# Christine8888/PsrSigSim

Hardware: AMD Instinct MI355X
Metric: channel-samples/sec (node) at 2048ch x 2^22 samp; % HBM roofline; speedup vs CPU (higher is better)
Workload: dtype f32

## Files before the change

psrsigsim_amd/csrc/pss_fourstep.hip:

```cpp
#include "pss_fourstep.hpp"

using namespace pss;

SideStreams *side_streams() {
    static SideStreams g[64];
    int dev = 0;
    if (hipGetDevice(&dev) != hipSuccess || dev < 0 || dev >= 64) return nullptr;
    SideStreams &x = g[dev];
    if (!x.ok) {
        for (int i = 0; i < 2; ++i)
            if (hipStreamCreateWithFlags(&x.s[i], hipStreamNonBlocking) != hipSuccess) return nullptr;
        for (int i = 0; i < 40; ++i)
            if (hipEventCreateWithFlags(&x.ev[i], hipEventDisableTiming) != hipSuccess) return nullptr;
        x.ok = true;
    }
    return &x;
}

__global__ __launch_bounds__(256) void k_mask_bits(KP k, uint32_t *bm) {
    const int r = blockIdx.y;
    const uint32_t j = blockIdx.x * 256u + threadIdx.x;
    const uint32_t wm = ((uint32_t)k.N - 1u) >> 5;
    if (j > wm) return;
    uint32_t is;
    float t;
    mask_split((uint64_t)k.p.mask_ramp[r], k.log2n, is, t);
    const uint32_t B = (uint32_t)k.mbB, RUN = B < 32u ? B : 32u;
    const uint32_t N1 = (uint32_t)k.N1, N2 = (uint32_t)k.N2;
    uint32_t out = 0;
    for (uint32_t s = 0; s < 32u; s += RUN) {
        const uint32_t bp = (j << 5) + s, e = bp / B, b = bp - e * B;
        const uint32_t n = (e % N1) * N2 + (e / N1) * B + b;
        out |= mask_run(k, n, is, t, RUN) << s;
    }
    bm[(int64_t)r * (wm + 1u) + j] = out;
}

__global__ __launch_bounds__(256) void k_mask_words(const uint2 *bits, uint32_t nwords, uint32_t *list,
                                                    uint32_t *count) {
    const uint32_t w = blockIdx.x * 256u + threadIdx.x;
    bool nz = false;
    if (w < nwords) {
        const uint2 b = bits[w];
        nz = (b.x | b.y) != 0u;
    }
    const uint64_t bal = __ballot(nz);
    const int lane = threadIdx.x & 63;
    uint32_t b0 = 0;
    if (lane == 0 && bal) b0 = atomicAdd(count, (uint32_t)__popcll(bal));
    b0 = __shfl(b0, 0);
    if (nz) list[b0 + (uint32_t)__popcll(bal & ((1ull << lane) - 1ull))] = w;
}

__global__ __launch_bounds__(256) void k_null_fix_list(KP k) {
    __shared__ uint32_t desc[4][64 * 9];
    __shared__ uint32_t dbase[4][64 * 9];
    const int r = blockIdx.y, lane = threadIdx.x & 63, wv = threadIdx.x >> 6;
    const PssPipeline &p = k.p;
    const uint32_t nl = *k.nwlist;
    const uint32_t nm = (uint32_t)k.N - 1u;
    uint32_t is;
    float t;
    mask_split((uint64_t)p.mask_ramp[r], k.log2n, is, t);
    const uint32_t c = (uint32_t)(p.chan0 + r);
    float *row = p.data + (int64_t)r * p.ld;
    const Rng gn(p.seed, p.call_noise, P_NOISE), gr(p.seed, p.call_null, P_REP);
    const float nn = p.noise_norm, sc = p.null_rep_scale;
    const uint32_t stride = gridDim.x * 256u;
    for (uint32_t i0 = blockIdx.x * 256u; i0 < nl; i0 += stride) {
        const uint32_t i = i0 + threadIdx.x;
        uint32_t hits = 0, n0 = 0;
        if (i < nl) {
            const uint32_t w = k.wlist[i];
            n0 = ((w << 5) + is) & nm;
            hits = mask_run(k, n0, is, t, 32u);
        }
        if (__ballot(hits != 0u) == 0ull) continue;
        const uint32_t a = n0 & 3u;
        const uint64_t hx = (uint64_t)hits << a;
        uint32_t cnt = 0;
#pragma unroll
        for (int g = 0; g < 9; ++g) cnt += ((uint32_t)(hx >> (4 * g)) & 15u) ? 1u : 0u;
        const uint64_t below = (1ull << lane) - 1ull;
        uint32_t e = 0, total = 0;
#pragma unroll
        for (int bit = 0; bit < 4; ++bit) {
            const uint64_t bal = __ballot((cnt >> bit) & 1u);
            e += (uint32_t)__popcll(bal & below) << bit;
            total += (uint32_t)__popcll(bal) << bit;
        }
#pragma unroll
        for (int g = 0; g < 9; ++g) {
            const uint32_t h = (uint32_t)(hx >> (4 * g)) & 15u;
            if (h) {
                desc[wv][e] = h;
                dbase[wv][e] = ((n0 - a) + 4u * (uint32_t)g) & nm;
                ++e;
            }
        }
        __builtin_amdgcn_fence(__ATOMIC_RELEASE, "wavefront");
        __builtin_amdgcn_wave_barrier();
        __builtin_amdgcn_fence(__ATOMIC_ACQUIRE, "wavefront");
        for (uint32_t e = (uint32_t)lane; e < total; e += 64u) {
            const uint32_t h = desc[wv][e], nb = dbase[wv][e];
            PSS_DASSERT((int64_t)nb + 4 <= k.N && (nb & 3u) == 0u);
            const float4 xn = chi2_1x4(gn.bits(nb >> 2, c, 0u));
            const float4 xr = chi2_1x4(gr.bits(nb >> 2, c, 0u));
            const float vn[4] = {xn.x, xn.y, xn.z, xn.w}, vr[4] = {xr.x, xr.y, xr.z, xr.w};
            if (h == 15u) {
                *reinterpret_cast<float4 *>(row + nb) =
                    make_float4(fmaf(nn, vn[0], vr[0] * sc), fmaf(nn, vn[1], vr[1] * sc),
                                fmaf(nn, vn[2], vr[2] * sc), fmaf(nn, vn[3], vr[3] * sc));
                continue;
            }
#pragma unroll
            for (int q = 0; q < 4; ++q)
                if ((h >> q) & 1u) row[nb + q] = fmaf(nn, vn[q], vr[q] * sc);
        }
        __builtin_amdgcn_fence(__ATOMIC_RELEASE, "wavefront");
        __builtin_amdgcn_wave_barrier();
        __builtin_amdgcn_fence(__ATOMIC_ACQUIRE, "wavefront");
    }
}

__global__ void k_node_params(uint64_t *ramp, float *nyq, int L) {
    const int j = threadIdx.x;
    if (j < KCH) {
        const double t = cospi((j + 0.5) / KCH);
        const double f = 0.5 * (t + 1.0);
        ramp[j] = (uint64_t)ldexp(f, 64 - L);
        nyq[j] = (float)cospi(f);
    }
}

__global__ __launch_bounds__(256) void k_mask_table(const float *nodes, int64_t N, uint2 *bits,
                                                    uint32_t *base, float *coef, uint32_t *counter) {
    __shared__ float T[KCH * KCH];
    if (threadIdx.x < KCH * KCH) {
        const int n = threadIdx.x / KCH, j = threadIdx.x - n * KCH;
        T[threadIdx.x] = (float)(cospi((double)n * (j + 0.5) / KCH) * (n ? 2.0 : 1.0) / KCH);
    }
    __syncthreads();
    const int64_t p = (int64_t)blockIdx.x * blockDim.x + threadIdx.x;
    float v[KCH], c[KCH];
#pragma unroll
    for (int j = 0; j < KCH; ++j) v[j] = nodes[(int64_t)j * N + p];
    float S = 0.f;
#pragma unroll
    for (int n = 0; n < KCH; ++n) {
        float s = 0.f;
#pragma unroll
        for (int j = 0; j < KCH; ++j) s = fmaf(T[n * KCH + j], v[j], s);
        c[n] = s;
        if (n) S += fabsf(s);
    }
    const float eps = 1e-3f + 4e-6f * (fabsf(c[0]) + S);
    const bool hi = c[0] - S > 1.0f + eps;
    const bool amb = !hi && !(c[0] + S < 1.0f - eps);
// ... 22 lines not shown
    for (uint32_t idx = blockIdx.x * 256u + threadIdx.x; idx < na; idx += gridDim.x * 256u) {
        float4 *dst = reinterpret_cast<float4 *>(coef + (int64_t)idx * KREC);
        const float4 q[3] = {dst[1], dst[2], dst[3]};
        const float c[KCH] = {q[0].x, q[0].y, q[0].z, q[0].w, q[1].x, q[1].y, q[1].z, q[1].w,
                              q[2].x, q[2].y, q[2].z, q[2].w};
        float S = 0.f;
#pragma unroll
        for (int n = 1; n < KCH; ++n) S += fabsf(c[n]);
        float D2 = 0.f;
#pragma unroll
        for (int n = 2; n < KCH; ++n) {
            const float n2 = (float)(n * n);
            D2 = fmaf(n2 * (n2 - 1.0f) * (1.0f / 3.0f), fabsf(c[n]), D2);
        }
        const float err = 4e-6f * (fabsf(c[0]) + S);
        constexpr int NG = 256;
        constexpr float H = 2.0f / NG;
        float rt[10];
#pragma unroll
        for (int i = 0; i < 10; ++i) rt[i] = INFINITY;
        float gprev = cheb_eval_r(q, -1.0f) - 1.0f;
        bool prev = gprev > 0.0f;
        const bool s0 = prev;
        bool cert = true;
        int cnt = 0;
        int jf[10];
#pragma unroll
        for (int i = 0; i < 10; ++i) jf[i] = 0;
        for (int jg = 1; jg <= NG; ++jg) {
            const float tg = -1.0f + (float)jg * H;
            const float g = cheb_eval_r(q, tg) - 1.0f;
            const bool cur = g > 0.0f;
            if (cur != prev) {
                cert = cert && (fabsf(g - gprev) - 2.0f * err > D2 * H * H);
#pragma unroll
                for (int i = 0; i < 10; ++i) if (i == cnt) jf[i] = jg;
                ++cnt;
            } else {
                cert = cert && (fminf(fabsf(g), fabsf(gprev)) - err > D2 * H * H * 0.125f);
            }
            prev = cur;
            gprev = g;
        }
        const int nb = cnt < 10 ? cnt : 10;
#pragma unroll
        for (int i = 0; i < 10; ++i) {
            if (i < nb) {
                const bool pv = (i & 1) ? !s0 : s0;
                float lo = -1.0f + (float)(jf[i] - 1) * H, hi = -1.0f + (float)jf[i] * H;
                for (int it = 0; it < 24; ++it) {
                    const float mid = 0.5f * (lo + hi);
                    if ((cheb_eval_r(q, mid) > 1.0f) == pv) lo = mid; else hi = mid;
                }
                rt[i] = lo;
            }
        }
        if (cert && cnt <= 10) {
            dst[0] = make_float4((float)cnt, s0 ? 1.0f : 0.0f, rt[0], rt[1]);
            dst[1] = make_float4(rt[2], rt[3], rt[4], rt[5]);
            dst[2] = make_float4(rt[6], rt[7], rt[8], rt[9]);
        } else {
            dst[0] = make_float4(-1.0f, 0.0f, 0.0f, 0.0f);
            dst[1] = q[0];
            dst[2] = q[1];
            dst[3] = q[2];
        }
    }
}

int launch_node_params(uint64_t *ramp, float *nyq, int L, hipStream_t st) {
    k_node_params<<<1, 64, 0, st>>>(ramp, nyq, L);
    LAUNCHCHK();
    return PSS_OK;
}
int launch_mask_table(const float *nodes, int64_t N, uint2 *bits, uint32_t *base, float *coef, uint32_t *counter,
                      hipStream_t st) {
    k_mask_table<<<dim3((unsigned)(N / 256)), dim3(256), 0, st>>>(nodes, N, bits, base, coef, counter);
    LAUNCHCHK();
    const unsigned gr = (unsigned)std::min<int64_t>(N / 256, 1024);
    k_mask_roots<<<dim3(gr), dim3(256), 0, st>>>(coef, counter);
    LAUNCHCHK();
    return PSS_OK;
}
int launch_mask_words(const uint2 *bits, uint32_t nwords, uint32_t *list, uint32_t *count, hipStream_t st) {
    k_mask_words<<<dim3((nwords + 255) / 256), dim3(256), 0, st>>>(bits, nwords, list, count);
    LAUNCHCHK();
    return PSS_OK;
}
int launch_mask_bits(const KP &k, uint32_t *bm, hipStream_t st) {
    k_mask_bits<<<dim3((unsigned)((k.N / 32 + 255) / 256), (unsigned)k.p.nchan), dim3(256), 0, st>>>(k, bm);
    LAUNCHCHK();
    return PSS_OK;
}
int launch_null_fix(const KP &k, hipStream_t st) {
    tk_begin(TK_NULLFIX, st);
    const unsigned gx = (unsigned)((k.N / 32 / 8 + 255) / 256);
    k_null_fix_list<<<dim3(gx ? gx : 1, (unsigned)k.p.nchan), dim3(256), 0, st>>>(k);
    tk_end(st);
    LAUNCHCHK();
    return PSS_OK;
}

int run_fourstep(KP &k, hipStream_t st, const float *mask_row) {
    if (!fourstep_split(k.N, plan_variant(k.p) == 0, &k.N1, &k.N2))
        return fail(PSS_EUNSUPPORTED, "four-step: N=%lld", (long long)k.N);
    plan_note("fourstep");
    if (k.N1 == 1024 && k.N2 == 4096) {
        return launch_pair<Pow2Split<1024, 4096>>(k, st, mask_row);
    }
    return run_fourstep_b(k, st, mask_row);
}
```

psrsigsim_amd/csrc/pss_fourstep.hpp:

```cpp
#pragma once
#include "pss_stages.hpp"
#include "pss_fft.hpp"


template <int N1, int B, int T, typename FWD>
struct Cols;

template <int N1, int B, int T, int... F>
struct Cols<N1, B, T, RList<F...>> {
    using FF = Fft<N1, B, T>;
    static constexpr int E = FF::E;
    static constexpr int RF0 = FF::template first<F...>();
    static constexpr int RFL = FF::template last_of<F...>();

    __device__ static void passA(const KP &k) {
        __shared__ cf lds[B * Lds<N1>::RS];
        const int tid = threadIdx.x;
        const int r = blockIdx.y;
        const int64_t n20 = (int64_t)blockIdx.x * B;
        const int64_t N2 = k.N2;
        const bool re_in = k.p.data_in_fft != 0;
        for (int it = tid; it < N1 * B / 4; it += T) {
            const int n1 = it / (B / 4);
            const int b4 = (it - n1 * (B / 4)) * 4;
// ... 830 lines not shown
        const uint32_t RP = (uint32_t)rpitch(k);
        const uint32_t s0 = (uint32_t)n20 * 8u;
        {
#pragma unroll 1
        for (int it = tid; it < N1 * B / 4; it += T) {
            const int k1 = it / (B / 4);
            const int b4 = (it - k1 * (B / 4)) * 4;
            const uint32_t off = ((uint32_t)k1 * RP + (uint32_t)b4) * 8u;
            const float4 lo = Y.ld4(off, s0), hi = Y.ld4(off + 16u, s0);
            const cf a[4] = {make_float2(lo.x, lo.y), make_float2(lo.z, lo.w),
                             make_float2(hi.x, hi.y), make_float2(hi.z, hi.w)};
            const uint32_t m0 = (uint32_t)(n20 + b4) * (uint32_t)k1;
            float r0 = (float)m0 * invN;
            if (r0 >= 0.5f) r0 -= 1.0f;
            float r1 = (float)k1 * invN;
            if (r1 >= 0.5f) r1 -= 1.0f;
            const cf w0 = expi_rev(r0), w1 = expi_rev(r1);
            const cf w2 = cmul(w1, w1);
            const cf tw[4] = {w0, cmul(w0, w1), cmul(w0, w2), cmul(w0, cmul(w2, w1))};
#pragma unroll
            for (int i = 0; i < 4; ++i) {
                lds[LdsC::at(b4 + i, k1)] = cmul(a[i], tw[i]);
            }
        }
        }
        __syncthreads();
        cf v[E];
        if constexpr (kWaveCols) {
            const int wv = tid >> 6, lane = tid & 63;
            cf *wl = lds + wv * LdsC::RS;
            FW::template load<RI0>(v, wl, lane);
            stage_sync<true>();
            FW::template run_tw<true, 1, I...>(v, wl, lane, tw16);
            FW::template store<RIL>(v, wl, lane);
        } else {
            FF::template load<RI0>(v, lds, tid);
            __syncthreads();
            FF::template run_tw<true, 1, I...>(v, lds, tid, tw16);
            FF::template store<RIL>(v, lds, tid);
        }
        __syncthreads();
    }

    __device__ static void passC(const KP &k) {
        __shared__ __align__(128) cf lds[B * LdsC::RS];
        const int tid = threadIdx.x;
        int cbx, pr;
        xcd_block(cbx, pr);
        const int ra = 2 * pr - k.poff, rb = ra + 1;
        const bool hasa = ra >= 0, hasb = rb < k.p.nchan;
        const int64_t n20 = (int64_t)cbx * B;
        const bool mask = k.mtab != 0;
        const float invN = k.invN;
        if constexpr (kRegCols) {
            cf x[N1];
            reg_unspill(k, x, pr, n20 + tid);
#pragma unroll
            for (int n1 = 0; n1 < N1; ++n1) lds[LdsC::at(tid, n1)] = x[n1];
            __syncthreads();
        } else {
            inv_block(k, k.Yd + (int64_t)pr * pstride(k), n20, lds, tid);
        }
#pragma unroll 1
        for (int it = tid; it < N1 * B / 4; it += T) {
            const int n1 = it / (B / 4);
            const int b4 = (it - n1 * (B / 4)) * 4;
            const int64_t n = n1 * k.N2 + n20 + b4;
            float da[4], db[4], ma[4], mb[4];
            const uint32_t ha = (mask && hasa) ? mask_bits4<B, N1>(k, ra, cbx, n1, b4) : 0u;
            const uint32_t hb = (mask && hasb) ? mask_bits4<B, N1>(k, rb, cbx, n1, b4) : 0u;
#pragma unroll
            for (int i = 0; i < 4; ++i) {
                const cf z = lds[LdsC::at(b4 + i, n1)];
                da[i] = z.x * invN;
                db[i] = z.y * invN;
                ma[i] = ((ha >> i) & 1u) ? 2.0f : 0.0f;
                mb[i] = ((hb >> i) & 1u) ? 2.0f : 0.0f;
            }
            if (hasa) epilogue4(k, ra, n, 4, da, ma, false);
            if (hasb) epilogue4(k, rb, n, 4, db, mb, false);
        }
    }

    __device__ static void passC_fast32(const KP &k) {
        static_assert((N1 == 1024 || N1 == 2048) && (T == 1024 || T == 512) && B % (T / 64) == 0 &&
                      kWaveCols == false, "register-resident wide pass C: 2^m columns of 1024 / 2048");
        constexpr int NW = T / 64, CPW = B / NW;
        constexpr int E1 = N1 / 64;
        constexpr int H = N1 / 2;
        constexpr int RSH = H + H / 16 + 1;
        constexpr int OSP = B + 1;
        using LW = Lds<N1, -1>;
        using FWC = Fft<N1, 1, 64, true, -1>;
        constexpr int RI0 = FWC::template first<I...>();
        constexpr int LRI = N1 / RI0;
        constexpr int B1 = B * RSH * 8, B2 = NW * LW::RS * 8, B3 = N1 * OSP * 4;
        constexpr int BUF = (B1 > B2 ? B1 : B2) > B3 ? (B1 > B2 ? B1 : B2) : B3;
        __shared__ __align__(16) char smem[BUF];
        __shared__ cf tw16[kTw16Size];
        const int tid = threadIdx.x, wv = tid >> 6, lane = tid & 63;
        tw16_fill(tw16, tid, T);
        int cbx, pr;
        xcd_block(cbx, pr);
        const int ra = 2 * pr - k.poff, rb = ra + 1;
        const bool hasa = ra >= 0, hasb = rb < k.p.nchan;
        const int64_t N2 = k.N2;
        const PssPipeline &p = k.p;
        const float invN = k.invN, nn = p.noise_norm;
        const int64_t n20 = (int64_t)cbx * B;
        const Buf Y(k.Yd + (int64_t)pr * pstride(k), (uint32_t)(pstride(k) * 8));
        const uint32_t RP = (uint32_t)rpitch(k);
        cf *hb = reinterpret_cast<cf *>(smem);
        cf v[CPW][E1];
        auto fresh = [](int x) __attribute__((always_inline)) { return N1 == 1024 ? opaque(x) : x; };
#pragma unroll
        for (int h = 0; h < 2; ++h) {
            if (h) __syncthreads();
#pragma unroll 1
            for (int it = tid; it < H * B / 4; it += T) {
                const int k1l = it / (B / 4), b4 = (it - k1l * (B / 4)) * 4;
                const int k1 = h * H + k1l;
                const uint32_t off = ((uint32_t)k1 * RP + (uint32_t)b4) * 8u, so = (uint32_t)n20 * 8u;
                const float4 lo = Y.ld4(off, so), hi = Y.ld4(off + 16u, so);
                const cf a[4] = {make_float2(lo.x, lo.y), make_float2(lo.z, lo.w),
                                 make_float2(hi.x, hi.y), make_float2(hi.z, hi.w)};
                const uint32_t m0 = (uint32_t)(n20 + b4) * (uint32_t)k1;
                float r0 = (float)m0 * invN;
                if (r0 >= 0.5f) r0 -= 1.0f;
                float r1 = (float)k1 * invN;
                if (r1 >= 0.5f) r1 -= 1.0f;
                const cf w0 = expi_rev(r0), w1 = expi_rev(r1);
                const cf w2 = cmul(w1, w1);
                const cf tw[4] = {w0, cmul(w0, w1), cmul(w0, w2), cmul(w0, cmul(w2, w1))};
#pragma unroll
                for (int i = 0; i < 4; ++i) hb[(b4 + i) * RSH + k1l + (k1l >> 4)] = cmul(a[i], tw[i]);
            }
            __syncthreads();
#pragma unroll
            for (int i = 0; i < E1; ++i) {
                const int pc = 64 * (i / RI0) + LRI * (i % RI0);
                if (pc / H != h) continue;
                const int pl = lane + pc - h * H;
#pragma unroll
                for (int c = 0; c < CPW; ++c) v[c][i] = hb[(wv + NW * c) * RSH + pl + (pl >> 4)];
            }
        }
        __syncthreads();
        {
            cf *wl = reinterpret_cast<cf *>(smem) + wv * LW::RS;
#pragma unroll
            for (int c = 0; c < CPW; ++c) {
                if (c) stage_sync<true>();
                FWC::template run_tw<true, 1, I...>(v[c], wl, fresh(lane), tw16);
            }
        }
        constexpr int RIL = FWC::template last_of<I...>();
        float *stg = reinterpret_cast<float *>(smem);
        const uint32_t ca = (uint32_t)(p.chan0 + ra), cb = ca + 1u;
        const Rng gn(p.seed, p.call_noise, P_NOISE);
        const uint32_t rbytes = (uint32_t)(k.N * 4);
#pragma unroll
        for (int ch = 0; ch < 2; ++ch) {
            __syncthreads();
            const int sl = fresh(lane);
#pragma unroll
            for (int i = 0; i < E1; ++i) {
                int bb, pos;
                FWC::template where<RIL>(i, sl, bb, pos);
#pragma unroll
                for (int c = 0; c < CPW; ++c) stg[pos * OSP + wv + NW * c] = (ch ? v[c][i].y : v[c][i].x) * invN;
            }
            __syncthreads();
            const bool has = ch ? hasb : hasa;
            if (!has) continue;
            const uint32_t c = ch ? cb : ca;
            const Buf o(p.data + (int64_t)(ch ? rb : ra) * p.ld, rbytes);
            const int t0 = fresh(tid);
#pragma unroll
            for (int t = 0; t < N1 * B / 4 / T; ++t) {
                const int it = t0 + t * T;
                const int n1 = it / (B / 4), c4 = (it - n1 * (B / 4)) * 4;
                const uint32_t n = (uint32_t)(n1 * (int)N2) + (uint32_t)n20 + (uint32_t)c4;
                const float4 x = chi2_1x4(gn.bits(n >> 2, c, 0u));
                const float *sr = stg + n1 * OSP + c4;
                o.st4(fmaf(nn, x.x, sr[0]), fmaf(nn, x.y, sr[1]), fmaf(nn, x.z, sr[2]), fmaf(nn, x.w, sr[3]),
                      n * 4u, 0);
            }
        }
    }

    __device__ static void passC_fast(const KP &k) {
        static_assert(kItemsExact, "fast pass C: whole items per thread");
        __shared__ __align__(128) cf lds[B * LdsC::RS];
        const int tid = threadIdx.x;
        int cbx, pr;
        xcd_block(cbx, pr);
        const int ra = 2 * pr - k.poff, rb = ra + 1;
        const bool hasa = ra >= 0, hasb = rb < k.p.nchan;
        const int64_t N2 = k.N2;
        const PssPipeline &p = k.p;
        const float invN = k.invN, nn = p.noise_norm;
        const uint32_t ca = (uint32_t)(p.chan0 + ra), cb = ca + 1u;
        const Rng gn(p.seed, p.call_noise, P_NOISE);
        const uint32_t rbytes = (uint32_t)(k.N * 4);
        const Buf oa(p.data + (int64_t)max(ra, 0) * p.ld, rbytes), ob(p.data + (int64_t)min(rb, p.nchan - 1) * p.ld, rbytes);
        const int64_t n20 = (int64_t)cbx * B;
        if constexpr (kRegCols) {
            cf x[N1];
            reg_unspill(k, x, pr, n20 + tid);
#pragma unroll
            for (int n1 = 0; n1 < N1; ++n1) lds[LdsC::at(tid, n1)] = x[n1];
            __syncthreads();
        } else {
            inv_block(k, k.Yd + (int64_t)pr * pstride(k), n20, lds, tid);
        }
        float acc[ITEMS][2][4];
#pragma unroll
        for (int t = 0; t < ITEMS; ++t) {
            const int it = tid + t * T;
            const int n1 = it / (B / 4);
            const int b4 = (it - n1 * (B / 4)) * 4;
            const uint32_t n = (uint32_t)(n1 * (int)N2) + (uint32_t)n20 + (uint32_t)b4;
            const float4 xa = chi2_1x4(gn.bits(n >> 2, ca, 0u));
            const float4 xb = chi2_1x4(gn.bits(n >> 2, cb, 0u));
            const float na[4] = {xa.x, xa.y, xa.z, xa.w}, nb[4] = {xb.x, xb.y, xb.z, xb.w};
#pragma unroll
            for (int i = 0; i < 4; ++i) {
                const cf z = lds[LdsC::at(b4 + i, n1)];
                acc[t][0][i] = fmaf(nn, na[i], z.x * invN);
                acc[t][1][i] = fmaf(nn, nb[i], z.y * invN);
            }
        }
#pragma unroll
        for (int t = 0; t < ITEMS; ++t) {
            const int it = tid + t * T;
            const int n1 = it / (B / 4);
            const int b4 = (it - n1 * (B / 4)) * 4;
            const uint32_t off = ((uint32_t)(n1 * (int)N2) + (uint32_t)n20 + (uint32_t)b4) * 4u;
            if (hasa) oa.st4(acc[t][0][0], acc[t][0][1], acc[t][0][2], acc[t][0][3], off, 0);
            if (hasb) ob.st4(acc[t][1][0], acc[t][1][1], acc[t][1][2], acc[t][1][3], off, 0);
        }
    }

    __device__ static void node_col(const KP &k, float *nodes) {
        __shared__ __align__(128) cf lds[B * LdsC::RS];
        const int tid = threadIdx.x;
        int cbx, pr;
        xcd_block(cbx, pr);
        const int64_t n20 = (int64_t)cbx * B;
        const float invN = k.invN;
        inv_block(k, k.Ym + (int64_t)pr * pstride(k), n20, lds, tid);
        float *ra = nodes + (int64_t)(2 * pr) * k.N, *rb = ra + k.N;
        for (int it = tid; it < N1 * B / 4; it += T) {
            const int n1 = it / (B / 4);
            const int b4 = (it - n1 * (B / 4)) * 4;
            const int64_t n = n1 * k.N2 + n20 + b4;
            float a[4], b[4];
#pragma unroll
            for (int i = 0; i < 4; ++i) {
                const cf z = lds[LdsC::at(b4 + i, n1)];
                a[i] = z.x * invN;
                b[i] = z.y * invN;
            }
            *reinterpret_cast<float4 *>(ra + n) = make_float4(a[0], a[1], a[2], a[3]);
            *reinterpret_cast<float4 *>(rb + n) = make_float4(b[0], b[1], b[2], b[3]);
        }
    }
};

template <typename C, int T>
__global__ __launch_bounds__(T) void k_pairA(KP k) { C::template passA<false>(k); }
template <typename C, int T, bool SHARED>
__global__ __launch_bounds__(T) void k_pairA_fast(KP k) { C::template passA<true, SHARED>(k); }
template <typename C>
__global__ __launch_bounds__(256) void k_prof_cols(KP k, float4 *out) { C::prof_cols(k, out); }
template <typename C, int T>
__global__ __launch_bounds__(T) void k_pairC(KP k) { C::passC(k); }
template <typename C, int T>
__global__ __launch_bounds__(T) void k_pairC_fast(KP k) { C::passC_fast(k); }
template <typename C, int T, int W = (T == 512 ? 2 : 4)>
__global__ __launch_bounds__(T, W) void k_pairC_fast32(KP k) { C::passC_fast32(k); }
template <typename C, int T>
__global__ __launch_bounds__(T) void k_node_col(KP k, float *nodes) { C::node_col(k, nodes); }
template <typename C, int T>
__global__ __launch_bounds__(T, C::kFoldWaves) void k_pairA_fold(KP k) { C::passA_fold(k); }
template <typename C, int T>
__global__ __launch_bounds__(T, C::kFoldWavesC) void k_pairC_fold(KP k) { C::passC_fold(k); }

constexpr int xrs_read(int B) { return B >= 32 ? 1 : 16; }

template <int N1_, int B_, int T_, typename CF, typename CI>
struct ColEngine {
    static constexpr int N1 = N1_, B = B_, T = T_;
    using PC = PairCols<N1, B, T, CF, CI, xrs_read(B)>;
    using PCFast = PairCols<N1, B, T, CF, CI, -1>;
    using PCFast32 = PairCols<N1, 16, 512, CF, CI, -1>;
    static constexpr int FB = B > 128 ? 128 : B;
    using PCFold = PairCols<N1, FB, FB, CF, CI>;
    using PCNode = PairCols<N1, B, T, CF, CI>;
    using MaskCols = Cols<N1, B, T, CF>;
};
template <int N1>
struct Pow2Cols;
template <> struct Pow2Cols<16> : ColEngine<16, 512, 512, C16, C16> {};
template <> struct Pow2Cols<32> : ColEngine<32, 256, 512, C32F, C32F> {};
template <> struct Pow2Cols<64> : ColEngine<64, 128, 512, C64F, C64F> {};
template <> struct Pow2Cols<128> : ColEngine<128, 64, 512, C128F, C128F> {};
template <> struct Pow2Cols<256> : ColEngine<256, 32, 512, C256, C256> {};
template <> struct Pow2Cols<512> : ColEngine<512, 16, 512, C512F, C512F> {};
template <> struct Pow2Cols<1024> : ColEngine<1024, 8, 512, C1kF, C1kF> {};
template <> struct Pow2Cols<2048> : ColEngine<2048, 8, 512, C2kF, C2kF> {};
template <int N1, typename CF, typename CI, int T>
using RegCols = ColEngine<N1, T, T, CF, CI>;

template <int N2_, int TR_, typename RF, typename RI, int TRF_>
struct RowEngine {
    static constexpr int N2 = N2_, TR = TR_, TRF = TRF_;
    using PR = PairRows<N2, TR, RF, RI>;
    static constexpr int TS = N2 / 16;
    using PRS = PairRowsSeq<N2, TS, RF, RI>;
    using MaskRows = Rows<N2, 1, TRF, RF>;
};
template <int N2>
struct RowsOf;
template <> struct RowsOf<1024> : RowEngine<1024, 128, C1kF, C1kI, 64> {};
template <> struct RowsOf<2048> : RowEngine<2048, 256, C2kF, C2kI, 128> {};
template <> struct RowsOf<4096> : RowEngine<4096, 512, C4k, C4k, 256> {};
template <> struct RowsOf<8192> : RowEngine<8192, 1024, C8kF, C8kI, 512> {};
template <> struct RowsOf<16384> : RowEngine<16384, 1024, C16kF, C16kI, 1024> {};
template <> struct RowsOf<2500> : RowEngine<2500, 250, RList<5, 5, 5, 5, 4>, RList<4, 5, 5, 5, 5>, 250> {};

template <typename C, typename R>
struct Split : C, R {
    static constexpr bool kMaskTable = (C::N1 & (C::N1 - 1)) == 0 && R::N2 <= 8192;
};
template <int N1, int N2>
using Pow2Split = Split<Pow2Cols<N1>, RowsOf<N2>>;

template <typename S>
static inline int build_mask_table(KP &k, hipStream_t st, const float *mask_row, char *w, const WsLayout &L) {
    constexpr int N1 = S::N1, N2 = S::N2, B = S::B, T = S::T, TR = S::TR, TRF = S::TRF;
    using PC = typename S::PCNode;
    using PR = typename S::PR;
    cf *mspec = reinterpret_cast<cf *>(w + L.mspec);
    uint32_t *counter = reinterpret_cast<uint32_t *>(w + L.misc);
    uint64_t *nramp = reinterpret_cast<uint64_t *>(w + L.misc + 64);
    float *nnyq = reinterpret_cast<float *>(w + L.misc + 192);
    float *nodes = reinterpret_cast<float *>(w + L.nodes);
    int log2n = 0;
    while ((1ll << log2n) < k.N) ++log2n;
    KP km = k;
    km.p.nchan = 1;
    km.p.chan0 = 0;
    km.p.data = const_cast<float *>(mask_row);
    km.p.ld = k.N;
    km.p.src = PSS_SRC_LOAD;
    km.p.null_mode = PSS_NULL_NONE;
    km.p.data_in_fft = 1;
    km.p.work = mspec;
    using C1 = typename S::MaskCols;
    using R1 = typename S::MaskRows;
    k_colA<C1, T><<<dim3((unsigned)(N2 / B), 1), dim3(T), 0, st>>>(km);
    LAUNCHCHK();
    k_row<R1, TRF><<<dim3((unsigned)N1, 1), dim3(TRF), 0, st>>>(km);
    LAUNCHCHK();
    if (const int rc = launch_node_params(nramp, nnyq, log2n, st)) return rc;
    KP kn = k;
    kn.p.nchan = KCH;
    kn.p.chan0 = 0;
    kn.p.ramp = nramp;
    kn.p.nyq_re = nnyq;
    kn.p.nyq_im = nnyq;
    kn.poff = 0;
    kn.npairs = KCH / 2;
    kn.Ym = reinterpret_cast<cf *>(w + L.ynode);
    kn.Mspec = mspec;
    k_node_row<PR, TR><<<dim3((unsigned)(KCH / 2), (unsigned)(N1 / 2)), dim3(TR), 0, st>>>(kn);
    LAUNCHCHK();
    k_node_col<PC, T><<<dim3((unsigned)(N2 / B), (unsigned)(KCH / 2)), dim3(T), 0, st>>>(kn, nodes);
    LAUNCHCHK();
    HIPCHK(hipMemsetAsync(counter, 0, 4, st));
    k.mt_bits = reinterpret_cast<const uint2 *>(w + L.bits);
    k.mt_base = reinterpret_cast<const uint32_t *>(w + L.base);
    k.mt_coef = reinterpret_cast<const float *>(w + L.coef);
    if (const int rc = launch_mask_table(nodes, k.N, reinterpret_cast<uint2 *>(w + L.bits),
                                         reinterpret_cast<uint32_t *>(w + L.base), reinterpret_cast<float *>(w + L.coef),
                                         counter, st))
        return rc;
    {
        uint32_t *wl = reinterpret_cast<uint32_t *>(w + L.wlist);
        uint32_t *wcount = reinterpret_cast<uint32_t *>(w + L.misc + 8);
        HIPCHK(hipMemsetAsync(wcount, 0, 4, st));
        const uint32_t nwords = (uint32_t)(k.N / 32);
        if (const int rc = launch_mask_words(k.mt_bits, nwords, wl, wcount, st)) return rc;
        k.wlist = wl;
        k.nwlist = wcount;
    }
    k.mtab = 1;
    plan_note(" N:table");
    k.log2n = log2n;
    if (k.p.data_in_fft && !fast_epilogue(k)) {
        k.mbB = B;
        uint32_t *bm = reinterpret_cast<uint32_t *>(w + L.mbits);
        if (const int rc = launch_mask_bits(k, bm, st)) return rc;
        k.mbits = bm;
    }
    return PSS_OK;
}

struct SideStreams {
    hipStream_t s[2];
    hipEvent_t ev[40];
    bool ok;
};
SideStreams *side_streams();

template <typename S>
static int fork_mask_table(KP &k, hipStream_t st, SideStreams *ss, const float *mask_row, char *w, const WsLayout &L) {
    if (ss) {
        HIPCHK(hipEventRecord(ss->ev[30], st));
        HIPCHK(hipStreamWaitEvent(ss->s[0], ss->ev[30], 0));
    }
    if (const int rc = build_mask_table<S>(k, ss ? ss->s[0] : st, mask_row, w, L)) return rc;
    if (ss) {
        HIPCHK(hipEventRecord(ss->ev[31], ss->s[0]));
        k.mask_ready = ss->ev[31];
    }
    return PSS_OK;
}

static constexpr int kMaskAfterANchan = 1024;

template <typename S>
static int launch_pair(KP &k, hipStream_t st, const float *mask_row) {
    constexpr int N1 = S::N1, N2 = S::N2, B = S::B, T = S::T, TR = S::TR;
    using PC = typename S::PC;
    using PR = typename S::PR;
    plan_note(" %dx%d", N1, N2);
    k.poff = k.p.chan0 & 1;
    k.npairs = (k.p.nchan + k.poff + 1) / 2;
    char *w = reinterpret_cast<char *>(k.p.work);
    const WsLayout L = ws_layout(k.p.nchan, k.N);
    k.Yd = reinterpret_cast<cf *>(w + L.yd);
    const bool table = k.p.null_mode == PSS_NULL_DELAYED;
    if (table && !S::kMaskTable)
        return fail(PSS_EUNSUPPORTED, "delayed null on the mixed-radix or 16384-row four-step (N=%lld)",
                    (long long)k.N);
    SideStreams *ss = table && k.p.data_in_fft ? side_streams() : nullptr;
    const bool table_after_a = ss && k.p.nchan <= kMaskAfterANchan;
    if constexpr (S::kMaskTable) {
        if (table && !table_after_a)
            if (const int rc = fork_mask_table<S>(k, st, ss, mask_row, w, L)) return rc;
    }
    if (!k.p.data_in_fft) {
        return launch_elementwise(k, st);
    }
    if (!k.p.htab) {
        cf *rt = reinterpret_cast<cf *>(w + L.rtab);
        k_pair_tab<PR::RFL><<<dim3((unsigned)k.npairs), dim3(64), 0, st>>>(k.p.ramp, k.N, k.p.nchan, k.poff,
                                                                          k.npairs, rt);
        LAUNCHCHK();
        k.rtab = rt;
    }

    const dim3 gc((unsigned)(N2 / B), (unsigned)k.npairs);
    tk_begin(TK_COLA, st);
    const bool fold_a = PC::kRegCols && fold_source(k.p);
    const bool fast_a = !fold_a && PC::kItemsExact && fast_source(k.p);
    if (fold_a) {
        if constexpr (PC::kRegCols) k_pairA_fold<PC, T><<<gc, dim3(T), 0, st>>>(k);
        plan_note(" A:fold");
    } else if (fast_a && k.p.prof_rows == 1) {
        if constexpr (PC::kItemsExact) {
            float4 *pcol = reinterpret_cast<float4 *>(w + L.pcol);
            const int64_t ne = k.N / 4;
            k_prof_cols<PC><<<dim3((unsigned)((ne + 255) / 256)), dim3(256), 0, st>>>(k, pcol);
            LAUNCHCHK();
            k.pcol = pcol;
            k_pairA_fast<PC, T, true><<<gc, dim3(T), 0, st>>>(k);
        }
        plan_note(" A:fast_shared");
    } else if (fast_a) {
        if constexpr (PC::kItemsExact) k_pairA_fast<PC, T, false><<<gc, dim3(T), 0, st>>>(k);
        plan_note(" A:fast");
    } else {
        k_pairA<PC, T><<<gc, dim3(T), 0, st>>>(k);
        plan_note(" A:generic");
    }
    tk_end(st);
    LAUNCHCHK();
    if constexpr (S::kMaskTable) {
        if (table_after_a)
            if (const int rc = fork_mask_table<S>(k, st, ss, mask_row, w, L)) return rc;
    }

    tk_begin(TK_ROW, st);
    const dim3 gr((unsigned)k.npairs, (unsigned)(N1 / 2));
    const bool plain = !k.p.htab && !k.p.tail_a;
    if (N2 > 8192 || (N2 == 8192 && plain)) {
        if (!plain) return fail(PSS_EUNSUPPORTED, "%d-point rows: no transfer function", N2);
        if constexpr (N2 >= 8192) {
            using PRS = typename S::PRS;
            constexpr int TS = S::TS;
            k_pair_row_seq<PRS, TS, false><<<dim3(gr.x, gr.y - 1), dim3(TS), 0, st>>>(k);
            k_pair_row_seq<PRS, TS, true><<<dim3(gr.x, 1u), dim3(TS), 0, st>>>(k);
        }
        plan_note(" R:pair_row_seq");
    } else if (k.p.htab) {
        if constexpr (N2 <= 8192) k_pair_row<PR, TR, false, true><<<gr, dim3(TR), 0, st>>>(k);
        plan_note(" R:pair_row_htab");
    } else if (k.p.tail_a) {
        if constexpr (N2 <= 8192) k_pair_row<PR, TR, true><<<gr, dim3(TR), 0, st>>>(k);
        plan_note(" R:pair_row_tail");
    } else {
        if constexpr (N2 < 8192) k_pair_row<PR, TR><<<gr, dim3(TR), 0, st>>>(k);
        plan_note(" R:pair_row");
    }
    tk_end(st);
    LAUNCHCHK();

    const bool fast = PC::kItemsExact && fast_epilogue(k);
    if (k.mask_ready && !fast) HIPCHK(hipStreamWaitEvent(st, k.mask_ready, 0));
    tk_begin(TK_COLC, st);
    if (fast) {
        const dim3 g16((unsigned)(N2 / 16), (unsigned)k.npairs);
        if constexpr (N1 == 2048) {
            k_pairC_fast32<typename S::PCFast32, 512><<<g16, dim3(512), 0, st>>>(k);
            plan_note(" C:fast32");
        } else if constexpr (N1 == 1024) {
            k_pairC_fast32<typename S::PCFast32, 512, 4><<<g16, dim3(512), 0, st>>>(k);
            plan_note(" C:fast C:cols16x2");
        } else if constexpr (PC::kItemsExact) {
            k_pairC_fast<typename S::PCFast, T><<<gc, dim3(T), 0, st>>>(k);
            plan_note(" C:fast");
        }
    } else if (PC::kRegCols && fold_epilogue(k)) {
        if constexpr (PC::kRegCols) {
            constexpr int FB = S::FB;
            k_pairC_fold<typename S::PCFold, FB><<<dim3((unsigned)(N2 / FB), gc.y), dim3(FB), 0, st>>>(k);
        }
        plan_note(" C:fold");
    } else {
        k_pairC<PC, T><<<gc, dim3(T), 0, st>>>(k);
        plan_note(" C:generic");
    }
    tk_end(st);
    LAUNCHCHK();

    if (fast && k.mtab) {
        if (k.mask_ready) HIPCHK(hipStreamWaitEvent(st, k.mask_ready, 0));
        if (const int rc = launch_null_fix(k, st)) return rc;
        plan_note(" N:fix_list");
    }
    return PSS_OK;
}

template <int N1, typename CF, typename CI, int T>
static int launch_smooth_n2(KP &k, hipStream_t st) {
    using C = RegCols<N1, CF, CI, T>;
    switch (k.N2) {
        case 1024: return launch_pair<Split<C, RowsOf<1024>>>(k, st, nullptr);
        case 2048: return launch_pair<Split<C, RowsOf<2048>>>(k, st, nullptr);
        case 4096: return launch_pair<Split<C, RowsOf<4096>>>(k, st, nullptr);
        case 8192: return launch_pair<Split<C, RowsOf<8192>>>(k, st, nullptr);
        default: return fail(PSS_EUNSUPPORTED, "mixed-radix four-step: N2=%lld", (long long)k.N2);
    }
}
```

psrsigsim_amd/csrc/pss_plan.hpp:

```cpp
#pragma once
#include <string.h>
#include <algorithm>

#include "pss_common.hpp"

using namespace pss;

enum { TK_ELEM = 0, TK_SINGLE, TK_COLA, TK_ROW, TK_COLC, TK_FALLBACK, TK_NULLFIX, TK_N };
void tk_begin(int kind, hipStream_t st);
void tk_end(hipStream_t st);
void plan_note(const char *fmt, ...);

struct KP {
    PssPipeline p;
    int64_t N;
    int64_t N1;
    int64_t N2;
    float invN;
    int npairs;
    int poff;
    cf *Yd;
    cf *Ym;
    const cf *Mspec;
    int mtab;
// ... 32 lines not shown
static inline bool smooth_col(int64_t n1) {
    switch (n1) {
        case 6: case 10: case 12: case 20: case 24: case 30: case 40: case 48: case 60: return true;
        default: return false;
    }
}
static inline bool smooth5_split(int64_t n, int64_t *N1 = nullptr, int64_t *N2 = nullptr) {
    if (n != 3125000) return false;
    if (N1) *N1 = 1250;
    if (N2) *N2 = 2500;
    return true;
}
static inline bool smooth_split(int64_t n, int64_t *N1 = nullptr, int64_t *N2 = nullptr) {
    if (smooth5_split(n, N1, N2)) return true;
    if (n <= 0 || (n & 1) || is_pow2(n) || n > (1ll << 24)) return false;
    int v2 = __builtin_ctzll((unsigned long long)n);
    const int m = v2 - 1 < 13 ? v2 - 1 : 13;
    if (m < 10) return false;
    const int64_t n2 = 1ll << m, n1 = n / n2;
    if (!smooth_col(n1)) return false;
    if (N1) *N1 = n1;
    if (N2) *N2 = n2;
    return true;
}

extern int g_flags;

struct BsGeom { int64_t M, M1, M2, nb; };
static inline bool bs_len(int64_t N) { return N > 8192 && N <= (1ll << 24); }
static inline BsGeom bs_geom(int32_t nchan, int64_t N) {
    BsGeom g;
    g.M = 1;
    while (g.M < 2 * N - 1) g.M <<= 1;
    g.M2 = g.M >= (1ll << 25) ? 8192 : 4096;
    g.M1 = g.M / g.M2;
    g.nb = ((int64_t)nchan * N + g.M - 1) / g.M;
    if (g.nb < 1) g.nb = 1;
    if (g.nb > nchan) g.nb = nchan;
    if (g.nb > 65535) g.nb = 65535;
    return g;
}

static inline int plan_variant(const PssPipeline &p) {
    return p.null_mode == PSS_NULL_DELAYED ? 1 : (p.htab || p.tail_a) ? 2 : 0;
}
static inline int plan_geometry(int64_t N, int variant, int64_t *N1 = nullptr, int64_t *N2 = nullptr) {
    int64_t n1 = 0, n2 = 0;
    int kind = PSS_PLAN_DIRECT;
    if (N <= 0 || (N & 1) || (N > (1ll << 24) && !is_pow2(N))) {
        kind = PSS_PLAN_UNSUPPORTED;
    } else if (is_pow2(N) && N >= 64 && N <= 8192) {
        kind = PSS_PLAN_SINGLE;
        n1 = 1;
        n2 = N;
    } else if (fourstep_split(N, variant == 0, &n1, &n2)) {
        kind = PSS_PLAN_FOURSTEP;
    } else if (variant != 1 && smooth_split(N, &n1, &n2)) {
        kind = PSS_PLAN_SMOOTH;
    } else if (bs_len(N) && !(g_flags & PSS_FLAG_DIRECT_DFT)) {
        const BsGeom g = bs_geom(1, N);
        kind = PSS_PLAN_BLUESTEIN;
        n1 = g.M1;
        n2 = g.M2;
    }
    if (N1) *N1 = n1;
    if (N2) *N2 = n2;
    return kind;
}

static constexpr int64_t kRefineMaxN = 1 << 17;
static constexpr int kBsParts = 16;
static inline int64_t refine_cap(int32_t nchan, int64_t N) {
    const int64_t all = (int64_t)nchan * N;
    return std::min<int64_t>(all, all / 8 + 65536);
}

struct WsLayout {
    int64_t yd, mspec, ynode, nodes, bits, base, coef, misc, mbits, rtab, wlist, row, total;
    int64_t bs_chirp, bs_bhat, bs_z;
    int64_t odd_tw;
    int64_t rf_tw, rf_B, rf_mx;
    int64_t rf_part, rf_list, rf_cnt;
    int64_t pcol;
};

static inline WsLayout ws_layout(int32_t nchan, int64_t N, bool filt = false) {
    WsLayout w;
    memset(&w, 0, sizeof(w));
    int64_t o = 0;
    auto refine_bufs = [&] {
        w.rf_tw = o; o += al256(N * 16);
        w.rf_B = o;  o += al256((N / 2 + 1) * 16);
        w.rf_mx = o; o += al256((int64_t)nchan * 4);
        w.rf_part = o; o += al256((int64_t)kBsParts * (N / 2 + 1) * 16);
        w.rf_list = o; o += al256(refine_cap(nchan, N) * 8);
        w.rf_cnt = o;  o += 256;
    };
    if (fourstep_len(N)) {
        const int64_t npairs = ((int64_t)nchan + 2) / 2;
        const int64_t ps = N;
        w.yd = o;    o += al256(npairs * ps * 8);
        w.mspec = o; o += al256(N * 8);
        w.ynode = o; o += al256((int64_t)(KCH / 2) * ps * 8);
        w.nodes = o; o += al256((int64_t)KCH * N * 4);
        w.bits = o;  o += al256((N / 32) * 8);
        w.base = o;  o += al256((N / 32) * 4);
        w.coef = o;  o += al256(N * KREC * 4);
        w.misc = o;  o += 256;
        w.mbits = o; o += al256((int64_t)nchan * (N / 8));
        w.rtab = o;  o += al256(npairs * 2 * 64 * 8);
        w.wlist = o; o += al256((N / 32) * 4);
        w.pcol = o;  o += al256(N * 4);
    } else if (!filt && is_pow2(N) && N >= 64 && N <= 8192) {
        o += al256((int64_t)nchan * N * 8);
        refine_bufs();
    } else {
        const bool odd = (N & 1) != 0;
        const bool w1_only = bs_len(N) && !odd && !smooth_split(N) && !(g_flags & PSS_FLAG_DIRECT_DFT);
        o += al256(w1_only ? (int64_t)nchan * N * 8 : 2 * (int64_t)nchan * N * 8 + N * 8);
        if (odd) {
            w.odd_tw = o;
            o += al256((N - 1) * 8);
        } else if (bs_len(N)) {
            const BsGeom g = bs_geom(nchan, N);
            w.bs_chirp = o; o += al256(N * 8);
            w.bs_bhat = o;  o += al256(g.M * 8);
            w.bs_z = o;     o += al256(g.nb * g.M * 8);
        }
        if (!odd && N <= kRefineMaxN) refine_bufs();
        if (smooth_split(N)) {
            const int64_t npairs = ((int64_t)nchan + 2) / 2;
            w.yd = 0;
            w.rtab = al256(npairs * N * 8);
            w.pcol = o; o += al256(N * 4);
        }
    }
    w.row = o;
    o += al256(N * 4);
    w.total = o;
    return w;
}

static inline bool refine_null(const KP &k) {
    return k.p.null_mode == PSS_NULL_DELAYED && (k.N & 1) == 0 && k.N <= kRefineMaxN && !k.p.tail_a &&
           !k.p.htab && !(g_flags & PSS_FLAG_NULL_F32);
}


static inline bool fast_source(const PssPipeline &p) {
    if (g_flags & PSS_FLAG_NO_FAST) return false;
    return p.src == PSS_SRC_SEARCH && !p.gen_amp && p.gen_df == 1.0f && !p.inj_gen && p.null_mode != PSS_NULL_UNDELAYED &&
           p.nint <= kFastNint && !p.prof_split && (uint32_t)p.nint == p.knot_m;
}
static inline bool fold_source(const PssPipeline &p) {
    if (g_flags & PSS_FLAG_NO_FAST) return false;
    return p.src == PSS_SRC_FOLD && !p.gen_amp && !p.inj_gen && p.gen_df != 1.0f && p.nph > 0 &&
           p.null_mode != PSS_NULL_UNDELAYED;
}
static inline bool fold_epilogue(const KP &k) {
    const PssPipeline &p = k.p;
    if (g_flags & PSS_FLAG_NO_FAST) return false;
    if (p.out_kind != PSS_OUT_NONE || p.inj_noise || p.inj_rep) return false;
    return p.noise && p.noise_df != 1.0f && p.null_mode != PSS_NULL_DELAYED;
}
static inline bool fast_epilogue(const KP &k) {
    const PssPipeline &p = k.p;
    if (g_flags & PSS_FLAG_NO_FAST) return false;
    if (p.out_kind != PSS_OUT_NONE || p.inj_noise || p.inj_rep) return false;
    if (!p.noise || p.noise_df != 1.0f) return false;
    if (p.null_mode == PSS_NULL_UNDELAYED) return false;
    if (p.null_mode == PSS_NULL_DELAYED && (!k.mtab || p.null_rep_df != 1.0f)) return false;
    return on_grid16(p.data, p.ld);
}

int launch_elementwise(const KP &k, hipStream_t st);
int launch_box_row(const KP &k, float *row, hipStream_t st);
int launch_null_fix(const KP &k, hipStream_t st);
int run_fourstep(KP &k, hipStream_t st, const float *mask_row);
int run_smooth(KP &k, hipStream_t st);
int run_smooth_b(KP &k, hipStream_t st);
int run_smooth_c(KP &k, hipStream_t st);
int run_fourstep_b(KP &k, hipStream_t st, const float *mask_row);
int run_single(KP &k, hipStream_t st);
int run_fallback(KP &k, hipStream_t st);
int launch_null_refine(KP &k, hipStream_t st);
int launch_fb_epilogue(KP &k, hipStream_t st);
int shift_rows_odd(float *rows, int32_t nrows, int64_t n, int64_t ld, const uint64_t *ramp, void *work,
                   hipStream_t st);
int launch_node_params(uint64_t *ramp, float *nyq, int L, hipStream_t st);
int launch_mask_table(const float *nodes, int64_t N, uint2 *bits, uint32_t *base, float *coef, uint32_t *counter,
                      hipStream_t st);
int launch_mask_words(const uint2 *bits, uint32_t nwords, uint32_t *list, uint32_t *count, hipStream_t st);
int launch_mask_bits(const KP &k, uint32_t *bm, hipStream_t st);
```

Before: 186.9 billion.

## Fuse null-mask replacement into fast column pass C, leave residual fix

Pass C for N1=1024 now reads the mask-table bits for each thread's column positions, builds a per-block list of masked 4-sample groups in shared memory, and writes the chi-square replacement values into staging before the store. A second word list of the mask-dependent words is built, so the separate null-fix kernel only processes those and launches with a smaller grid. This removes most of the global read-modify-write traffic of the null-fix pass. In exchange, pass C must wait on the mask event earlier and carries extra shared memory, registers, and atomics. The new list reuses the nodes buffer, which may be unsafe if that buffer is still live.

```diff
diff --git a/psrsigsim_amd/csrc/pss_fourstep.hip b/psrsigsim_amd/csrc/pss_fourstep.hip
--- a/psrsigsim_amd/csrc/pss_fourstep.hip
+++ b/psrsigsim_amd/csrc/pss_fourstep.hip
@@ -37,21 +37,27 @@
 }
 
 __global__ __launch_bounds__(256) void k_mask_words(const uint2 *bits, uint32_t nwords, uint32_t *list,
-                                                    uint32_t *count) {
+                                                    uint32_t *count, uint32_t *list_f, uint32_t *count_f) {
     const uint32_t w = blockIdx.x * 256u + threadIdx.x;
-    bool nz = false;
+    bool nz = false, fd = false;
     if (w < nwords) {
         const uint2 b = bits[w];
         nz = (b.x | b.y) != 0u;
-    }
-    const uint64_t bal = __ballot(nz);
+        fd = b.y != 0u;
+    }
+    const uint64_t bal = __ballot(nz), balf = __ballot(fd);
     const int lane = threadIdx.x & 63;
-    uint32_t b0 = 0;
+    const uint64_t below = (1ull << lane) - 1ull;
+    uint32_t b0 = 0, f0 = 0;
     if (lane == 0 && bal) b0 = atomicAdd(count, (uint32_t)__popcll(bal));
+    if (lane == 0 && balf) f0 = atomicAdd(count_f, (uint32_t)__popcll(balf));
     b0 = __shfl(b0, 0);
-    if (nz) list[b0 + (uint32_t)__popcll(bal & ((1ull << lane) - 1ull))] = w;
-}
-
+    f0 = __shfl(f0, 0);
+    if (nz) list[b0 + (uint32_t)__popcll(bal & below)] = w;
+    if (fd) list_f[f0 + (uint32_t)__popcll(balf & below)] = w;
+}
+
+template <bool FDEP>
 __global__ __launch_bounds__(256) void k_null_fix_list(KP k) {
     __shared__ uint32_t desc[4][64 * 9];
     __shared__ uint32_t dbase[4][64 * 9];
@@ -74,6 +80,7 @@
             const uint32_t w = k.wlist[i];
             n0 = ((w << 5) + is) & nm;
             hits = mask_run(k, n0, is, t, 32u);
+            if (FDEP) hits &= k.mt_bits[w].y;
         }
         if (__ballot(hits != 0u) == 0ull) continue;
         const uint32_t a = n0 & 3u;
@@ -262,8 +269,9 @@
     LAUNCHCHK();
     return PSS_OK;
 }
-int launch_mask_words(const uint2 *bits, uint32_t nwords, uint32_t *list, uint32_t *count, hipStream_t st) {
-    k_mask_words<<<dim3((nwords + 255) / 256), dim3(256), 0, st>>>(bits, nwords, list, count);
+int launch_mask_words(const uint2 *bits, uint32_t nwords, uint32_t *list, uint32_t *count, uint32_t *list_f,
+                      uint32_t *count_f, hipStream_t st) {
+    k_mask_words<<<dim3((nwords + 255) / 256), dim3(256), 0, st>>>(bits, nwords, list, count, list_f, count_f);
     LAUNCHCHK();
     return PSS_OK;
 }
@@ -272,10 +280,12 @@
     LAUNCHCHK();
     return PSS_OK;
 }
-int launch_null_fix(const KP &k, hipStream_t st) {
+int launch_null_fix(const KP &k, hipStream_t st, bool fdep) {
     tk_begin(TK_NULLFIX, st);
-    const unsigned gx = (unsigned)((k.N / 32 / 8 + 255) / 256);
-    k_null_fix_list<<<dim3(gx ? gx : 1, (unsigned)k.p.nchan), dim3(256), 0, st>>>(k);
+    const unsigned gx = (unsigned)((k.N / 32 / (fdep ? 64 : 8) + 255) / 256);
+    const dim3 g(gx ? gx : 1, (unsigned)k.p.nchan);
+    if (fdep) k_null_fix_list<true><<<g, dim3(256), 0, st>>>(k);
+    else k_null_fix_list<false><<<g, dim3(256), 0, st>>>(k);
     tk_end(st);
     LAUNCHCHK();
     return PSS_OK;
diff --git a/psrsigsim_amd/csrc/pss_fourstep.hpp b/psrsigsim_amd/csrc/pss_fourstep.hpp
--- a/psrsigsim_amd/csrc/pss_fourstep.hpp
+++ b/psrsigsim_amd/csrc/pss_fourstep.hpp
@@ -936,6 +936,7 @@
         }
     }
 
+    template <bool NULLC = false>
     __device__ static void passC_fast32(const KP &k) {
         static_assert((N1 == 1024 || N1 == 2048) && (T == 1024 || T == 512) && B % (T / 64) == 0 &&
                       kWaveCols == false, "register-resident wide pass C: 2^m columns of 1024 / 2048");
@@ -952,8 +953,14 @@
         constexpr int BUF = (B1 > B2 ? B1 : B2) > B3 ? (B1 > B2 ? B1 : B2) : B3;
         __shared__ __align__(16) char smem[BUF];
         __shared__ cf tw16[kTw16Size];
+        static_assert(!NULLC || (N1 == 1024 && T == 512 && B == 16), "NULLC: two rows per thread, 16-bit entries");
+        __shared__ uint16_t nlist[NULLC ? N1 * B / 4 : 1];
+        __shared__ uint32_t ncount[2];
         const int tid = threadIdx.x, wv = tid >> 6, lane = tid & 63;
         tw16_fill(tw16, tid, T);
+        if constexpr (NULLC) {
+            if (tid < 2) ncount[tid] = 0u;
+        }
         int cbx, pr;
         xcd_block(cbx, pr);
         const int ra = 2 * pr - k.poff, rb = ra + 1;
@@ -966,6 +973,28 @@
         const uint32_t RP = (uint32_t)rpitch(k);
         cf *hb = reinterpret_cast<cf *>(smem);
         cf v[CPW][E1];
+        uint32_t mlo[2][N1 / T] = {}, mhi[2][N1 / T] = {}, msh[2][N1 / T] = {}, nwin[2] = {0u, 0u};
+        if constexpr (NULLC) {
+#pragma unroll
+            for (int ch = 0; ch < 2; ++ch) {
+                if (ch ? hasb : hasa) {
+                    uint32_t is;
+                    float tf;
+                    mask_split((uint64_t)p.mask_ramp[ch ? rb : ra], k.log2n, is, tf);
+                    const uint32_t nm = (uint32_t)k.N - 1u, wm = nm >> 5;
+                    const uint32_t *ax = reinterpret_cast<const uint32_t *>(k.mt_bits);
+#pragma unroll
+                    for (int j = 0; j < N1 / T; ++j) {
+                        const uint32_t p0 = ((uint32_t)(tid + j * T) * (uint32_t)N2 + (uint32_t)n20 - is) & nm;
+                        const uint32_t w = p0 >> 5;
+                        PSS_DASSERT(w <= wm);
+                        mlo[ch][j] = ax[2u * w];
+                        mhi[ch][j] = ax[2u * ((w + 1u) & wm)];
+                        msh[ch][j] = p0 & 31u;
+                    }
+                }
+            }
+        }
         auto fresh = [](int x) __attribute__((always_inline)) { return N1 == 1024 ? opaque(x) : x; };
 #pragma unroll
         for (int h = 0; h < 2; ++h) {
@@ -1000,6 +1029,14 @@
             }
         }
         __syncthreads();
+        if constexpr (NULLC) {
+#pragma unroll
+            for (int ch = 0; ch < 2; ++ch)
+#pragma unroll
+                for (int j = 0; j < N1 / T; ++j)
+                    nwin[ch] |= ((uint32_t)(((((uint64_t)mhi[ch][j]) << 32) | mlo[ch][j]) >> msh[ch][j]) & 0xffffu)
+                                << (16 * j);
+        }
         {
             cf *wl = reinterpret_cast<cf *>(smem) + wv * LW::RS;
 #pragma unroll
@@ -1024,10 +1061,61 @@
 #pragma unroll
                 for (int c = 0; c < CPW; ++c) stg[pos * OSP + wv + NW * c] = (ch ? v[c][i].y : v[c][i].x) * invN;
             }
+            if constexpr (NULLC) {
+                if (ch ? hasb : hasa) {
+                    uint32_t win[N1 / T], cnt = 0;
+#pragma unroll
+                    for (int j = 0; j < N1 / T; ++j) {
+                        win[j] = (nwin[ch] >> (16 * j)) & 0xffffu;
+#pragma unroll
+                        for (int g = 0; g < 4; ++g) cnt += ((win[j] >> (4 * g)) & 15u) ? 1u : 0u;
+                    }
+                    const uint64_t below = (1ull << lane) - 1ull;
+                    uint32_t e = 0, total = 0;
+#pragma unroll
+                    for (int bit = 0; bit < 4; ++bit) {
+                        const uint64_t bal = __ballot((cnt >> bit) & 1u);
+                        e += (uint32_t)__popcll(bal & below) << bit;
+                        total += (uint32_t)__popcll(bal) << bit;
+                    }
+                    uint32_t b0 = 0;
+                    if (lane == 0 && total) b0 = atomicAdd(&ncount[ch], total);
+                    e += (uint32_t)__shfl((int)b0, 0);
+                    const uint32_t r0 = (uint32_t)fresh(tid);
+#pragma unroll
+                    for (int j = 0; j < N1 / T; ++j) {
+#pragma unroll
+                        for (int g = 0; g < 4; ++g) {
+                            const uint32_t h = (win[j] >> (4 * g)) & 15u;
+                            if (h) {
+                                PSS_DASSERT(e < (uint32_t)(N1 * B / 4));
+                                nlist[e++] = (uint16_t)(((r0 + (uint32_t)(j * T)) << 6) | ((uint32_t)g << 4) | h);
+                            }
+                        }
+                    }
+                }
+            }
             __syncthreads();
             const bool has = ch ? hasb : hasa;
             if (!has) continue;
             const uint32_t c = ch ? cb : ca;
+            if constexpr (NULLC) {
+                const uint32_t ne = ncount[ch];
+                const Rng gr(p.seed, p.call_null, P_REP);
+                const float sc = p.null_rep_scale;
+                for (uint32_t e = (uint32_t)fresh(tid); e < ne; e += (uint32_t)T) {
+                    const uint32_t d = nlist[e], n1 = d >> 6, c4 = ((d >> 4) & 3u) * 4u;
+                    const uint32_t nb = n1 * (uint32_t)N2 + (uint32_t)n20 + c4;
+                    PSS_DASSERT(n1 < (uint32_t)N1 && (int64_t)nb + 4 <= k.N);
+                    const float4 xr = chi2_1x4(gr.bits(nb >> 2, c, 0u));
+                    float *sr = stg + n1 * OSP + c4;
+                    if (d & 1u) sr[0] = xr.x * sc;
+                    if (d & 2u) sr[1] = xr.y * sc;
+                    if (d & 4u) sr[2] = xr.z * sc;
+                    if (d & 8u) sr[3] = xr.w * sc;
+                }
+                __syncthreads();
+            }
             const Buf o(p.data + (int64_t)(ch ? rb : ra) * p.ld, rbytes);
             const int t0 = fresh(tid);
 #pragma unroll
@@ -1134,6 +1222,8 @@
 __global__ __launch_bounds__(T) void k_pairC_fast(KP k) { C::passC_fast(k); }
 template <typename C, int T, int W = (T == 512 ? 2 : 4)>
 __global__ __launch_bounds__(T, W) void k_pairC_fast32(KP k) { C::passC_fast32(k); }
+template <typename C>
+__global__ __launch_bounds__(512, 4) void k_pairC_null(KP k) { C::template passC_fast32<true>(k); }
 template <typename C, int T>
 __global__ __launch_bounds__(T) void k_node_col(KP k, float *nodes) { C::node_col(k, nodes); }
 template <typename C, int T>
@@ -1244,9 +1334,11 @@
     {
         uint32_t *wl = reinterpret_cast<uint32_t *>(w + L.wlist);
         uint32_t *wcount = reinterpret_cast<uint32_t *>(w + L.misc + 8);
-        HIPCHK(hipMemsetAsync(wcount, 0, 4, st));
         const uint32_t nwords = (uint32_t)(k.N / 32);
-        if (const int rc = launch_mask_words(k.mt_bits, nwords, wl, wcount, st)) return rc;
+        uint32_t *wlf = reinterpret_cast<uint32_t *>(w + L.wlist_f);
+        uint32_t *wcount_f = reinterpret_cast<uint32_t *>(w + L.wcount_f);
+        HIPCHK(hipMemsetAsync(wcount, 0, 8, st));
+        if (const int rc = launch_mask_words(k.mt_bits, nwords, wl, wcount, wlf, wcount_f, st)) return rc;
         k.wlist = wl;
         k.nwlist = wcount;
     }
@@ -1374,7 +1466,8 @@
     LAUNCHCHK();
 
     const bool fast = PC::kItemsExact && fast_epilogue(k);
-    if (k.mask_ready && !fast) HIPCHK(hipStreamWaitEvent(st, k.mask_ready, 0));
+    const bool nullc = fast && N1 == 1024 && S::kMaskTable && k.mtab;
+    if (k.mask_ready && (!fast || nullc)) HIPCHK(hipStreamWaitEvent(st, k.mask_ready, 0));
     tk_begin(TK_COLC, st);
     if (fast) {
         const dim3 g16((unsigned)(N2 / 16), (unsigned)k.npairs);
@@ -1382,8 +1475,9 @@
             k_pairC_fast32<typename S::PCFast32, 512><<<g16, dim3(512), 0, st>>>(k);
             plan_note(" C:fast32");
         } else if constexpr (N1 == 1024) {
-            k_pairC_fast32<typename S::PCFast32, 512, 4><<<g16, dim3(512), 0, st>>>(k);
-            plan_note(" C:fast C:cols16x2");
+            if (nullc) k_pairC_null<typename S::PCFast32><<<g16, dim3(512), 0, st>>>(k);
+            else k_pairC_fast32<typename S::PCFast32, 512, 4><<<g16, dim3(512), 0, st>>>(k);
+            plan_note(nullc ? " C:fast C:cols16x2 C:null" : " C:fast C:cols16x2");
         } else if constexpr (PC::kItemsExact) {
             k_pairC_fast<typename S::PCFast, T><<<gc, dim3(T), 0, st>>>(k);
             plan_note(" C:fast");
@@ -1402,8 +1496,13 @@
     LAUNCHCHK();
 
     if (fast && k.mtab) {
-        if (k.mask_ready) HIPCHK(hipStreamWaitEvent(st, k.mask_ready, 0));
-        if (const int rc = launch_null_fix(k, st)) return rc;
+        if (k.mask_ready && !nullc) HIPCHK(hipStreamWaitEvent(st, k.mask_ready, 0));
+        KP kf = k;
+        if (nullc) {
+            kf.wlist = reinterpret_cast<const uint32_t *>(w + L.wlist_f);
+            kf.nwlist = reinterpret_cast<const uint32_t *>(w + L.wcount_f);
+        }
+        if (const int rc = launch_null_fix(kf, st, nullc)) return rc;
         plan_note(" N:fix_list");
     }
     return PSS_OK;
diff --git a/psrsigsim_amd/csrc/pss_plan.hpp b/psrsigsim_amd/csrc/pss_plan.hpp
--- a/psrsigsim_amd/csrc/pss_plan.hpp
+++ b/psrsigsim_amd/csrc/pss_plan.hpp
@@ -138,6 +138,7 @@
     int64_t rf_tw, rf_B, rf_mx;
     int64_t rf_part, rf_list, rf_cnt;
     int64_t pcol;
+    int64_t wlist_f, wcount_f;
 };
 
 static inline WsLayout ws_layout(int32_t nchan, int64_t N, bool filt = false) {
@@ -163,6 +164,8 @@
         w.base = o;  o += al256((N / 32) * 4);
         w.coef = o;  o += al256(N * KREC * 4);
         w.misc = o;  o += 256;
+        w.wlist_f = w.nodes;
+        w.wcount_f = w.misc + 12;
         w.mbits = o; o += al256((int64_t)nchan * (N / 8));
         w.rtab = o;  o += al256(npairs * 2 * 64 * 8);
         w.wlist = o; o += al256((N / 32) * 4);
@@ -231,7 +234,7 @@
 
 int launch_elementwise(const KP &k, hipStream_t st);
 int launch_box_row(const KP &k, float *row, hipStream_t st);
-int launch_null_fix(const KP &k, hipStream_t st);
+int launch_null_fix(const KP &k, hipStream_t st, bool fdep);
 int run_fourstep(KP &k, hipStream_t st, const float *mask_row);
 int run_smooth(KP &k, hipStream_t st);
 int run_smooth_b(KP &k, hipStream_t st);
@@ -246,5 +249,6 @@
 int launch_node_params(uint64_t *ramp, float *nyq, int L, hipStream_t st);
 int launch_mask_table(const float *nodes, int64_t N, uint2 *bits, uint32_t *base, float *coef, uint32_t *counter,
                       hipStream_t st);
-int launch_mask_words(const uint2 *bits, uint32_t nwords, uint32_t *list, uint32_t *count, hipStream_t st);
+int launch_mask_words(const uint2 *bits, uint32_t nwords, uint32_t *list, uint32_t *count, uint32_t *list_f,
+                      uint32_t *count_f, hipStream_t st);
 int launch_mask_bits(const KP &k, uint32_t *bm, hipStream_t st);
```

After: 189.8 billion, median of 6. +1.5%, better.
